# hmmlillian/Neural-Color-Transfer

Hardware: AMD Instinct MI355X
Metric: 700x700 pairs/sec end-to-end L=5->1; PatchMatch HBM GB/s vs peak (higher is better)
Workload: dtype f32

## Files before the change

### neural-color-transfer_amd/csrc/k_vgg.hip

```cpp
#include "nct_internal.h"
#include "nct_device.h"

typedef float f32x16 __attribute__((ext_vector_type(16)));

__global__ void k_vgg_preprocess(const uint8_t* __restrict__ bgr, int stride, float* __restrict__ out, int H, int W) {
    int i = blockIdx.x * blockDim.x + threadIdx.x;
    if (i >= H * W) return;
    int y = i / W, x = i - y * W;
    const uint8_t* p = bgr + (size_t)y * stride + x * 3;
    out[i] = (float)p[0] - 103.939f;
    out[(size_t)H * W + i] = (float)p[1] - 116.779f;
    out[(size_t)2 * H * W + i] = (float)p[2] - 123.68f;
    out[(size_t)3 * H * W + i] = 0.f;
}

struct ConvGeom { int Cin, Cout, H, W, npx_blocks, nblk_n, tiles_x, Ho, Wo; };
#ifndef NCT_CONV_PT1_BELOW
#define NCT_CONV_PT1_BELOW 128
#endif

typedef float f32x32 __attribute__((ext_vector_type(32)));
typedef uint32_t u32x3 __attribute__((ext_vector_type(3)));

template <int WCO, int CT, bool POOL>
__device__ __forceinline__ void conv3x3_mfma2b_body(const float* __restrict__ in, const float* __restrict__ wp ,
                                                    const float* __restrict__ bias, float* __restrict__ out, const ConvGeom& g, int relu, float* __restrict__ out_hwc, int bid) {
    constexpr int WPX = 4 / WCO;
    constexpr int BLK_PX = WPX * 64;
    constexpr int BLK_CO = WCO * 32 * CT;
    const int HW = g.H * g.W;
    int pt, nb;
    {
        const int grp = bid / (8 * g.nblk_n), rem = bid - grp * 8 * g.nblk_n;
        nb = rem >> 3; pt = grp * 8 + (rem & 7);
    }
    if (pt >= g.npx_blocks) return;
    const int wave = threadIdx.x >> 6, lane = threadIdx.x & 63;
    const int half = lane >> 5, l31 = lane & 31;
    const int wco = wave % WCO, wpx = wave / WCO;
    const int m0 = nb * BLK_CO + wco * 32 * CT;
    int y, x, tile_y = 0, tile_x = 0; bool live;
    if constexpr (POOL) {
        const int wt = pt * WPX + wpx;
        tile_y = wt / g.tiles_x; tile_x = wt - tile_y * g.tiles_x;
        y = 2 * tile_y + half; x = 32 * tile_x + l31;
        live = y < g.H && x < g.W;
    } else {
        const int p = pt * BLK_PX + wpx * 64 + lane;
        live = p < HW;
        const int pc = live ? p : 0;
        y = pc / g.W; x = pc - y * g.W;
    }
    const int bias_px = g.H >= 2 ? g.W + 1 : 1;
    const unsigned plane_bytes = (unsigned)HW * 4u, bias_bytes = (unsigned)bias_px * 4u;
    const auto rs = __builtin_amdgcn_make_buffer_rsrc((void*)in, 0, (unsigned)g.Cin * plane_bytes, 0x00020000);

    unsigned voff[3];
    bool rowv[3];
#pragma unroll
    for (int r = 0; r < 3; ++r) {
        voff[r] = live ? (unsigned)(((y + r - 1) * g.W + x - 1 + bias_px) * 4) : 0xFFF00000u;
        rowv[r] = live && (y + r - 1) >= 0 && (y + r - 1) < g.H;
    }
    const bool xl = x > 0, xr = x < g.W - 1;
    auto tapv = [&](int r, int d) { return d == 0 ? (rowv[r] && xl) : (d == 2 ? (rowv[r] && xr) : rowv[r]); };
    bool tm[9];
#pragma unroll
    for (int t = 0; t < 9; ++t) tm[t] = tapv(t / 3, t % 3);

    const float4* ap4 = reinterpret_cast<const float4*>(wp) + (size_t)half * g.Cout + m0 + l31;
    const float* ap1 = wp + (size_t)16 * g.Cout + (size_t)half * g.Cout + m0 + l31;
    unsigned soff = plane_bytes - bias_bytes;

    f32x32 acc0 = {0}, acc1 = {0};
    struct ASet { float4 q0, q1; float s8; };
    struct BSet { u32x3 r[2][3]; };
    ASet a0x, a1x, a0y, a1y; BSet bx, by;
    auto bload = [&](unsigned so, int r) { return __builtin_amdgcn_raw_buffer_load_b96(rs, voff[r], so, 0); };
#ifndef NCT_CONV_TIMING_SKIP
#define NCT_CONV_TIMING_SKIP 0
#endif
    auto load_pair = [&](ASet& a0, ASet& a1, BSet& b) {
        constexpr bool LA = !(NCT_CONV_TIMING_SKIP & 1), LB = !(NCT_CONV_TIMING_SKIP & 2);
        if constexpr (LA) {
            a0.q0 = ap4[0]; a0.q1 = ap4[(size_t)2 * g.Cout]; a0.s8 = ap1[0];
            if constexpr (CT == 2) { a1.q0 = ap4[32]; a1.q1 = ap4[(size_t)2 * g.Cout + 32]; a1.s8 = ap1[32]; }
        }
        if constexpr (LB) {
#pragma unroll
            for (int r = 0; r < 3; ++r) { b.r[0][r] = bload(soff - plane_bytes, r); b.r[1][r] = bload(soff, r); }
        }
        ap4 += (size_t)18 * g.Cout / 4;
        ap1 += (size_t)18 * g.Cout;
        soff += 2u * plane_bytes;
    };
    auto aval = [](const ASet& a, int s) -> float {
        switch (s) { case 0: return a.q0.x; case 1: return a.q0.y; case 2: return a.q0.z; case 3: return a.q0.w;
                     case 4: return a.q1.x; case 5: return a.q1.y; case 6: return a.q1.z; case 7: return a.q1.w; default: return a.s8; }
    };
    auto mma_pair = [&](const ASet& a0, const ASet& a1, const BSet& b) {
#pragma unroll
        for (int k = 0; k < 18; ++k) {
            const int ci = k / 9, t = k - 9 * ci, r = t / 3, d = t - 3 * r, s = k >> 1;
            const float bv = tm[t] ? __uint_as_float(b.r[ci][r][d]) : 0.f;
            if (k & 1) {
                acc0 = __builtin_amdgcn_mfma_f32_32x32x1f32(aval(a0, s), bv, acc0, 1, 1, 0);
                if constexpr (CT == 2) acc1 = __builtin_amdgcn_mfma_f32_32x32x1f32(aval(a1, s), bv, acc1, 1, 1, 0);
            } else {
                acc0 = __builtin_amdgcn_mfma_f32_32x32x1f32(aval(a0, s), bv, acc0, 1, 0, 0);
                if constexpr (CT == 2) acc1 = __builtin_amdgcn_mfma_f32_32x32x1f32(aval(a1, s), bv, acc1, 1, 0, 0);
            }
        }
    };
#ifndef NCT_CONV_SCHED
#define NCT_CONV_SCHED 0
#endif
    auto interleave = [] {
        if constexpr (NCT_CONV_SCHED == 2) return;
        if constexpr (CT == 2) {
#pragma unroll
            for (int i = 0; i < 12; ++i) {
                __builtin_amdgcn_sched_group_barrier(0x008, NCT_CONV_SCHED == 1 ? 1 : 2, 0);
                __builtin_amdgcn_sched_group_barrier(0x020, 1, 0);
                __builtin_amdgcn_sched_group_barrier(0x008, NCT_CONV_SCHED == 1 ? 2 : 1, 0);
            }
        } else {
#pragma unroll
            for (int i = 0; i < 9; ++i) {
                __builtin_amdgcn_sched_group_barrier(0x008, 1, 0);
                __builtin_amdgcn_sched_group_barrier(0x020, 1, 0);
                __builtin_amdgcn_sched_group_barrier(0x008, 1, 0);
            }
        }
    };
    {
        a0x.q0 = ap4[0]; a0x.q1 = ap4[(size_t)2 * g.Cout]; a0x.s8 = ap1[0];
        if constexpr (CT == 2) { a1x.q0 = ap4[32]; a1x.q1 = ap4[(size_t)2 * g.Cout + 32]; a1x.s8 = ap1[32]; }
        ap4 += (size_t)18 * g.Cout / 4;
        ap1 += (size_t)18 * g.Cout;
#pragma unroll
        for (int r = 0; r < 3; ++r) {
            const unsigned v0 = voff[r] - bias_bytes + (xl ? 0u : 4u);
            u32x3 t = __builtin_amdgcn_raw_buffer_load_b96(rs, v0, 0, 0);
            if (!xl) { t.z = t.y; t.y = t.x; }
            bx.r[0][r] = t;
            bx.r[1][r] = __builtin_amdgcn_raw_buffer_load_b96(rs, voff[r], soff, 0);
        }
        soff += 2u * plane_bytes;
    }
    int c2 = 0;
    for (; c2 + 4 <= g.Cin; c2 += 4) {
        load_pair(a0y, a1y, by);
        mma_pair(a0x, a1x, bx);
        interleave();
        __builtin_amdgcn_sched_barrier(0);
        if (c2 + 4 >= g.Cin) { ap4 -= (size_t)18 * g.Cout / 4; ap1 -= (size_t)18 * g.Cout; soff -= 2u * plane_bytes; }
        load_pair(a0x, a1x, bx);
        mma_pair(a0y, a1y, by);
        interleave();
        __builtin_amdgcn_sched_barrier(0);
    }
    if (c2 < g.Cin) mma_pair(a0x, a1x, bx);

    if constexpr (POOL) {
        const int xx = 32 * tile_x + l31, y0 = 2 * tile_y;
        const bool ok0 = y0 < g.H && xx < g.W, ok1 = y0 + 1 < g.H && xx < g.W;
        const size_t po = (size_t)tile_y * g.Wo + (xx >> 1), pn = (size_t)g.Ho * g.Wo;
        const bool writer = ok0 && !(l31 & 1);
        auto pool4 = [&](float top, float bot) {
            top = ok0 ? top : -3.402823466e+38f; bot = ok1 ? bot : -3.402823466e+38f;
            const float top_r = dpp_rot<0xB1>(top), bot_r = dpp_rot<0xB1>(bot);
            float m = -3.402823466e+38f;
            m = top > m ? top : m; m = top_r > m ? top_r : m; m = bot > m ? bot : m; m = bot_r > m ? bot_r : m;
            return m;
        };
#pragma unroll
        for (int r = 0; r < 16; ++r) {
            const int co0 = m0 + (r & 3) + 8 * (r >> 2) + 4 * half;
            const float bb0 = bias[co0];
            float t0 = acc0[r] + bb0, u0 = acc0[16 + r] + bb0;
            if (relu) { t0 = fmaxf(t0, 0.f); u0 = fmaxf(u0, 0.f); }
            const float m0v = pool4(t0, u0);
            if (writer) out[(size_t)co0 * pn + po] = m0v;
            if constexpr (CT == 2) {
                const float bb1 = bias[co0 + 32];
                float t1 = acc1[r] + bb1, u1 = acc1[16 + r] + bb1;
                if (relu) { t1 = fmaxf(t1, 0.f); u1 = fmaxf(u1, 0.f); }
                const float m1v = pool4(t1, u1);
                if (writer) out[(size_t)(co0 + 32) * pn + po] = m1v;
            }
        }
    } else {
        const int pw = pt * BLK_PX + wpx * 64;
        if (out_hwc) {
#pragma unroll
            for (int b = 0; b < 2; ++b) {
                const int pp = pw + 32 * b + l31;
                if (pp < HW) {
                    float* dst = out_hwc + (size_t)pp * g.Cout + m0 + 4 * half;
#pragma unroll
                    for (int gq = 0; gq < 4; ++gq) {
                        float4 v0, v1;
                        float* e0 = &v0.x; float* e1 = &v1.x;
#pragma unroll
                        for (int j = 0; j < 4; ++j) {
                            const int row = j + 8 * gq + 4 * half;
                            float t0 = acc0[16 * b + 4 * gq + j] + bias[m0 + row];
                            if (relu) t0 = fmaxf(t0, 0.f);
                            e0[j] = t0;
                            if constexpr (CT == 2) { float t1 = acc1[16 * b + 4 * gq + j] + bias[m0 + 32 + row]; if (relu) t1 = fmaxf(t1, 0.f); e1[j] = t1; }
                        }
                        *reinterpret_cast<float4*>(dst + 8 * gq) = v0;
                        if constexpr (CT == 2) *reinterpret_cast<float4*>(dst + 32 + 8 * gq) = v1;
                    }
                }
            }
        }
        if (out)
#pragma unroll
        for (int b = 0; b < 2; ++b) {
            const int pp = pw + 32 * b + l31;
            const bool lv = pp < HW;
#pragma unroll
            for (int r = 0; r < 16; ++r) {
                const int row = (r & 3) + 8 * (r >> 2) + 4 * half;
                const int co0 = m0 + row;
                float v0 = acc0[16 * b + r] + bias[co0];
                if (relu) v0 = fmaxf(v0, 0.f);
                if (lv) out[(size_t)co0 * HW + pp] = v0;
                if constexpr (CT == 2) {
                    float v1 = acc1[16 * b + r] + bias[co0 + 32];
                    if (relu) v1 = fmaxf(v1, 0.f);
                    if (lv) out[(size_t)(co0 + 32) * HW + pp] = v1;
                }
            }
        }
    }
}

bool nctk_conv3x3_pool_fits(int H, int W) {
    const long t2 = (long)cdiv(W, 32) * cdiv(H, 2), t1 = cdiv(H * W, 64);
    return t2 * 100 <= t1 * 104;
}

template <int WCO, int CT, bool POOL>
__global__ __launch_bounds__(256) __attribute__((amdgpu_waves_per_eu(3, 3))) void k_conv3x3_mfma2b(const float* __restrict__ in, const float* __restrict__ wp, const float* __restrict__ bias,
                                                        float* __restrict__ out, ConvGeom g, int relu, float* __restrict__ out_hwc) {
    conv3x3_mfma2b_body<WCO, CT, POOL>(in, wp, bias, out, g, relu, out_hwc, (int)blockIdx.x);
}
template <int WCO, int CT>
__global__ __launch_bounds__(256) __attribute__((amdgpu_waves_per_eu(3, 3))) void k_conv3x3_mfma2b_pair(const float* __restrict__ in1, const float* __restrict__ in2, const float* __restrict__ wp,
                                                        const float* __restrict__ bias, float* __restrict__ out1, float* __restrict__ out2, ConvGeom g1, ConvGeom g2, int nblocks1, int relu,
                                                        float* __restrict__ hwc1, float* __restrict__ hwc2) {
    const bool second = (int)blockIdx.x >= nblocks1;
    conv3x3_mfma2b_body<WCO, CT, false>(second ? in2 : in1, wp, bias, second ? out2 : out1, second ? g2 : g1, relu, second ? hwc2 : hwc1, second ? (int)blockIdx.x - nblocks1 : (int)blockIdx.x);
}
int nctk_conv3x3(nct_ctx* ctx, hipStream_t s, const float* in, const float* wp, const float* bias, float* out,
                 int Cin, int Cout, int H, int W, int relu, int pool, float* out_hwc) {
    NCT_REQUIRE(out || out_hwc, "conv3x3: no output");
    NCT_REQUIRE(!(pool && out_hwc), "conv3x3: the channel-last output exists for un-pooled layers only");
    NCT_REQUIRE((Cin & 1) == 0 && (Cout & 63) == 0, "conv3x3: Cin=%d must be even (pad) and Cout=%d a multiple of 64", Cin, Cout);
    NCT_REQUIRE((size_t)Cin * H * W * 4 < ((size_t)1 << 32), "conv3x3: input of %d x %d x %d floats exceeds the 4 GB a buffer descriptor addresses", Cin, H, W);
    const int WCO = (Cout % 128 == 0) ? 2 : 1;
    const int tiles_x = cdiv(W, 32), ntiles = pool ? tiles_x * cdiv(H, 2) : cdiv(H * W, 64);
    const int full_blocks = cdiv(ntiles, 4 / WCO) * (Cout / (64 * WCO));
    const int Ho = (H - 1) / 2 + 1, Wo = (W - 1) / 2 + 1;
#define NCT_CONV_LAUNCH(wco, ct, wpx, nblk_n_)                                                                                                    \
    do {                                                                                                                                          \
        ConvGeom g{Cin, Cout, H, W, cdiv(ntiles, wpx), nblk_n_, tiles_x, Ho, Wo};                                                                  \
        const int nblocks = cdiv(g.npx_blocks, 8) * 8 * g.nblk_n;                                                                                 \
        if (pool) hipLaunchKernelGGL((k_conv3x3_mfma2b<wco, ct, true>), dim3(nblocks), dim3(256), 0, s, in, wp, bias, out, g, relu, (float*)nullptr);             \
        else      hipLaunchKernelGGL((k_conv3x3_mfma2b<wco, ct, false>), dim3(nblocks), dim3(256), 0, s, in, wp, bias, out, g, relu, out_hwc);            \
    } while (0)
    if (full_blocks >= NCT_CONV_PT1_BELOW) {
        if (WCO == 2) NCT_CONV_LAUNCH(2, 2, 2, Cout / 128);
        else          NCT_CONV_LAUNCH(1, 2, 4, Cout / 64);
    } else if (Cout % 128 == 0) NCT_CONV_LAUNCH(4, 1, 1, Cout / 128);
    else                        NCT_CONV_LAUNCH(2, 1, 2, Cout / 64);
#undef NCT_CONV_LAUNCH
    NCT_LAUNCH_CHECK();
    return 0;
}

int nctk_conv3x3_pair(nct_ctx* ctx, hipStream_t s, const float* in1, int H1, int W1, const float* in2, int H2, int W2, const float* wp, const float* bias,
                      float* out1, float* out2, int Cin, int Cout, int relu, float* hwc1, float* hwc2) {
    auto small = [&](int H, int W) {
        const int WCO = (Cout % 128 == 0) ? 2 : 1;
        return cdiv(cdiv(H * W, 64), 4 / WCO) * (Cout / (64 * WCO)) < NCT_CONV_PT1_BELOW;
    };
    const bool ok = (Cin & 1) == 0 && (Cout & 63) == 0 && small(H1, W1) && small(H2, W2) && (size_t)Cin * H1 * W1 * 4 < ((size_t)1 << 32) && (size_t)Cin * H2 * W2 * 4 < ((size_t)1 << 32) &&
                    (out1 || hwc1) && (out2 || hwc2) && ctx->conv_pair != 0;
    if (!ok) {
        int rc = nctk_conv3x3(ctx, s, in1, wp, bias, out1, Cin, Cout, H1, W1, relu, 0, hwc1); if (rc) return rc;
        return nctk_conv3x3(ctx, s, in2, wp, bias, out2, Cin, Cout, H2, W2, relu, 0, hwc2);
    }
    const int nt1 = cdiv(H1 * W1, 64), nt2 = cdiv(H2 * W2, 64);
#define NCT_CONV_PAIR(wco, ct, wpx, nblk_n_)                                                                                                      \
    do {                                                                                                                                          \
        ConvGeom g1{Cin, Cout, H1, W1, cdiv(nt1, wpx), nblk_n_, 0, 0, 0}, g2{Cin, Cout, H2, W2, cdiv(nt2, wpx), nblk_n_, 0, 0, 0};                 \
        const int nb1 = cdiv(g1.npx_blocks, 8) * 8 * g1.nblk_n, nb2 = cdiv(g2.npx_blocks, 8) * 8 * g2.nblk_n;                                     \
        hipLaunchKernelGGL((k_conv3x3_mfma2b_pair<wco, ct>), dim3(nb1 + nb2), dim3(256), 0, s, in1, in2, wp, bias, out1, out2, g1, g2, nb1, relu, hwc1, hwc2); \
    } while (0)
    if (Cout % 128 == 0) NCT_CONV_PAIR(4, 1, 1, Cout / 128);
    else                 NCT_CONV_PAIR(2, 1, 2, Cout / 64);
#undef NCT_CONV_PAIR
    NCT_LAUNCH_CHECK();
    return 0;
}

__global__ void k_maxpool2x2(const float* __restrict__ in, float* __restrict__ out, int C, int H, int W, int Ho, int Wo) {
    size_t i = (size_t)blockIdx.x * blockDim.x + threadIdx.x;
    if (i >= (size_t)C * Ho * Wo) return;
    const int px = (int)(i % Wo); const size_t t = i / Wo; const int py = (int)(t % Ho); const int c = (int)(t / Ho);
    const int hs = py * 2, ws = px * 2, he = min(hs + 2, H), we = min(ws + 2, W);
    const float* p = in + (size_t)c * H * W;
    float m = -3.402823466e+38f;
    for (int y = hs; y < he; ++y)
        for (int x = ws; x < we; ++x) { const float v = p[(size_t)y * W + x]; m = v > m ? v : m; }
    out[i] = m;
}

int nctk_maxpool2x2(nct_ctx* ctx, hipStream_t s, const float* in, float* out, int C, int H, int W) {
    const int Ho = (H - 2 + 1) / 2 + 1, Wo = (W - 2 + 1) / 2 + 1;
    const size_t n = (size_t)C * Ho * Wo;
    hipLaunchKernelGGL(k_maxpool2x2, dim3((unsigned)((n + 255) / 256)), dim3(256), 0, s, in, out, C, H, W, Ho, Wo);
    NCT_LAUNCH_CHECK();
    return 0;
}

int nctk_vgg_preprocess(nct_ctx* ctx, hipStream_t s, const uint8_t* bgr, int stride, float* out, int H, int W) {
    hipLaunchKernelGGL(k_vgg_preprocess, dim3(cdiv(H * W, 256)), dim3(256), 0, s, bgr, stride, out, H, W);
    NCT_LAUNCH_CHECK();
    return 0;
}

__global__ void k_pack_weights(const float* __restrict__ w, float* __restrict__ wp, int Cout, int Cin, int Cin_pad) {
    size_t i = (size_t)blockIdx.x * blockDim.x + threadIdx.x;
    if (i >= (size_t)Cin_pad * 9 * Cout) return;
    const int co = (int)(i % Cout); const int k = (int)(i / Cout);
    const int ci = k / 9, tap = k - ci * 9;
    const float v = ci < Cin ? w[((size_t)co * Cin + ci) * 9 + tap] : 0.f;
    const int P = ci >> 1, k18 = (ci & 1) * 9 + tap, s_ = k18 >> 1, h = k18 & 1;
    const size_t base = (size_t)P * 18 * Cout;
    const size_t dst = s_ < 8 ? base + (size_t)(s_ >> 2) * 8 * Cout + ((size_t)h * Cout + co) * 4 + (s_ & 3)
                              : base + (size_t)16 * Cout + (size_t)h * Cout + co;
    wp[dst] = v;
}

int nctk_pack_weights(nct_ctx* ctx, hipStream_t s, const float* w, float* wp, int Cout, int Cin, int Cin_pad) {
    const size_t n = (size_t)Cin_pad * 9 * Cout;
    hipLaunchKernelGGL(k_pack_weights, dim3((unsigned)((n + 255) / 256)), dim3(256), 0, s, w, wp, Cout, Cin, Cin_pad);
    NCT_LAUNCH_CHECK();
    return 0;
}
```

Baseline: 15.76.

## Deepen conv3x3 MFMA load pipeline to configurable depth with buffer-load weights

Replaces the two-stage ping-pong prefetch in the 3x3 conv MFMA kernel with a D-stage register ring (default 3), so loads for pair p+D-1 are issued while pair p is multiplied. Weight fetches move from pointer arithmetic to buffer-descriptor loads with computed offsets, and a clamp replaces the end-of-loop pointer rewind. Occupancy is lowered from 3 to 2 waves per EU to make room for the extra staged registers. The aim is to hide more memory latency, at the cost of fewer resident waves and more register use.

```diff
diff --git a/neural-color-transfer_amd/csrc/k_vgg.hip b/neural-color-transfer_amd/csrc/k_vgg.hip
--- a/neural-color-transfer_amd/csrc/k_vgg.hip
+++ b/neural-color-transfer_amd/csrc/k_vgg.hip
@@ -1,5 +1,7 @@
 #include "nct_internal.h"
 #include "nct_device.h"
+#include <type_traits>
+#include <utility>
 
 typedef float f32x16 __attribute__((ext_vector_type(16)));
 
@@ -22,7 +24,10 @@
 typedef float f32x32 __attribute__((ext_vector_type(32)));
 typedef uint32_t u32x3 __attribute__((ext_vector_type(3)));
 
-template <int WCO, int CT, bool POOL>
+template <typename F, int... J> __device__ __forceinline__ void static_for_(F&& f, std::integer_sequence<int, J...>) { (f(std::integral_constant<int, J>{}), ...); }
+template <int N, typename F> __device__ __forceinline__ void static_for(F&& f) { static_for_(f, std::make_integer_sequence<int, N>{}); }
+
+template <int WCO, int CT, bool POOL, int D>
 __device__ __forceinline__ void conv3x3_mfma2b_body(const float* __restrict__ in, const float* __restrict__ wp ,
                                                     const float* __restrict__ bias, float* __restrict__ out, const ConvGeom& g, int relu, float* __restrict__ out_hwc, int bid) {
     constexpr int WPX = 4 / WCO;
@@ -68,47 +73,57 @@
 #pragma unroll
     for (int t = 0; t < 9; ++t) tm[t] = tapv(t / 3, t % 3);
 
-    const float4* ap4 = reinterpret_cast<const float4*>(wp) + (size_t)half * g.Cout + m0 + l31;
-    const float* ap1 = wp + (size_t)16 * g.Cout + (size_t)half * g.Cout + m0 + l31;
-    unsigned soff = plane_bytes - bias_bytes;
+    const int npairs = g.Cin >> 1;
+    const unsigned wpair_bytes = 72u * (unsigned)g.Cout;
+    const auto wrs = __builtin_amdgcn_make_buffer_rsrc((void*)wp, 0, (unsigned)npairs * wpair_bytes, 0x00020000);
+    const unsigned wq = (unsigned)(half * g.Cout + m0 + l31) * 16u;
+    const unsigned w8 = (unsigned)(half * g.Cout + m0 + l31) * 4u + 64u * (unsigned)g.Cout;
+    const unsigned wq1 = 32u * (unsigned)g.Cout;
 
     f32x32 acc0 = {0}, acc1 = {0};
     struct ASet { float4 q0, q1; float s8; };
-    struct BSet { u32x3 r[2][3]; };
-    ASet a0x, a1x, a0y, a1y; BSet bx, by;
-    auto bload = [&](unsigned so, int r) { return __builtin_amdgcn_raw_buffer_load_b96(rs, voff[r], so, 0); };
+    struct OSet { ASet a[CT]; u32x3 b[2][3]; };
+    OSet st[D];
+    auto wload4 = [&](unsigned vo, unsigned so) { return __builtin_bit_cast(float4, __builtin_amdgcn_raw_buffer_load_b128(wrs, vo, so, 0)); };
+    auto wload1 = [&](unsigned vo, unsigned so) { return __uint_as_float(__builtin_amdgcn_raw_buffer_load_b32(wrs, vo, so, 0)); };
+    auto aload = [&](ASet& a, int t, unsigned so) {
+        a.q0 = wload4(wq + 512u * t, so); a.q1 = wload4(wq + wq1 + 512u * t, so); a.s8 = wload1(w8 + 128u * t, so);
+    };
 #ifndef NCT_CONV_TIMING_SKIP
 #define NCT_CONV_TIMING_SKIP 0
 #endif
-    auto load_pair = [&](ASet& a0, ASet& a1, BSet& b) {
+    auto load_pair = [&](OSet& o, int p) {
         constexpr bool LA = !(NCT_CONV_TIMING_SKIP & 1), LB = !(NCT_CONV_TIMING_SKIP & 2);
+        p = min(p, npairs - 1);
         if constexpr (LA) {
-            a0.q0 = ap4[0]; a0.q1 = ap4[(size_t)2 * g.Cout]; a0.s8 = ap1[0];
-            if constexpr (CT == 2) { a1.q0 = ap4[32]; a1.q1 = ap4[(size_t)2 * g.Cout + 32]; a1.s8 = ap1[32]; }
+            const unsigned so = (unsigned)p * wpair_bytes;
+#pragma unroll
+            for (int t = 0; t < CT; ++t) aload(o.a[t], t, so);
         }
         if constexpr (LB) {
-#pragma unroll
-            for (int r = 0; r < 3; ++r) { b.r[0][r] = bload(soff - plane_bytes, r); b.r[1][r] = bload(soff, r); }
-        }
-        ap4 += (size_t)18 * g.Cout / 4;
-        ap1 += (size_t)18 * g.Cout;
-        soff += 2u * plane_bytes;
+            const unsigned so = (unsigned)(2 * p + 1) * plane_bytes - bias_bytes;
+#pragma unroll
+            for (int r = 0; r < 3; ++r) {
+                o.b[0][r] = __builtin_amdgcn_raw_buffer_load_b96(rs, voff[r], so - plane_bytes, 0);
+                o.b[1][r] = __builtin_amdgcn_raw_buffer_load_b96(rs, voff[r], so, 0);
+            }
+        }
     };
     auto aval = [](const ASet& a, int s) -> float {
         switch (s) { case 0: return a.q0.x; case 1: return a.q0.y; case 2: return a.q0.z; case 3: return a.q0.w;
                      case 4: return a.q1.x; case 5: return a.q1.y; case 6: return a.q1.z; case 7: return a.q1.w; default: return a.s8; }
     };
-    auto mma_pair = [&](const ASet& a0, const ASet& a1, const BSet& b) {
+    auto mma_pair = [&](const OSet& o) {
 #pragma unroll
         for (int k = 0; k < 18; ++k) {
             const int ci = k / 9, t = k - 9 * ci, r = t / 3, d = t - 3 * r, s = k >> 1;
-            const float bv = tm[t] ? __uint_as_float(b.r[ci][r][d]) : 0.f;
+            const float bv = tm[t] ? __uint_as_float(o.b[ci][r][d]) : 0.f;
             if (k & 1) {
-                acc0 = __builtin_amdgcn_mfma_f32_32x32x1f32(aval(a0, s), bv, acc0, 1, 1, 0);
-                if constexpr (CT == 2) acc1 = __builtin_amdgcn_mfma_f32_32x32x1f32(aval(a1, s), bv, acc1, 1, 1, 0);
+                acc0 = __builtin_amdgcn_mfma_f32_32x32x1f32(aval(o.a[0], s), bv, acc0, 1, 1, 0);
+                if constexpr (CT == 2) acc1 = __builtin_amdgcn_mfma_f32_32x32x1f32(aval(o.a[CT - 1], s), bv, acc1, 1, 1, 0);
             } else {
-                acc0 = __builtin_amdgcn_mfma_f32_32x32x1f32(aval(a0, s), bv, acc0, 1, 0, 0);
-                if constexpr (CT == 2) acc1 = __builtin_amdgcn_mfma_f32_32x32x1f32(aval(a1, s), bv, acc1, 1, 0, 0);
+                acc0 = __builtin_amdgcn_mfma_f32_32x32x1f32(aval(o.a[0], s), bv, acc0, 1, 0, 0);
+                if constexpr (CT == 2) acc1 = __builtin_amdgcn_mfma_f32_32x32x1f32(aval(o.a[CT - 1], s), bv, acc1, 1, 0, 0);
             }
         }
     };
@@ -134,33 +149,28 @@
         }
     };
     {
-        a0x.q0 = ap4[0]; a0x.q1 = ap4[(size_t)2 * g.Cout]; a0x.s8 = ap1[0];
-        if constexpr (CT == 2) { a1x.q0 = ap4[32]; a1x.q1 = ap4[(size_t)2 * g.Cout + 32]; a1x.s8 = ap1[32]; }
-        ap4 += (size_t)18 * g.Cout / 4;
-        ap1 += (size_t)18 * g.Cout;
+#pragma unroll
+        for (int t = 0; t < CT; ++t) aload(st[0].a[t], t, 0u);
 #pragma unroll
         for (int r = 0; r < 3; ++r) {
             const unsigned v0 = voff[r] - bias_bytes + (xl ? 0u : 4u);
             u32x3 t = __builtin_amdgcn_raw_buffer_load_b96(rs, v0, 0, 0);
             if (!xl) { t.z = t.y; t.y = t.x; }
-            bx.r[0][r] = t;
-            bx.r[1][r] = __builtin_amdgcn_raw_buffer_load_b96(rs, voff[r], soff, 0);
-        }
-        soff += 2u * plane_bytes;
-    }
-    int c2 = 0;
-    for (; c2 + 4 <= g.Cin; c2 += 4) {
-        load_pair(a0y, a1y, by);
-        mma_pair(a0x, a1x, bx);
-        interleave();
-        __builtin_amdgcn_sched_barrier(0);
-        if (c2 + 4 >= g.Cin) { ap4 -= (size_t)18 * g.Cout / 4; ap1 -= (size_t)18 * g.Cout; soff -= 2u * plane_bytes; }
-        load_pair(a0x, a1x, bx);
-        mma_pair(a0y, a1y, by);
-        interleave();
-        __builtin_amdgcn_sched_barrier(0);
-    }
-    if (c2 < g.Cin) mma_pair(a0x, a1x, bx);
+            st[0].b[0][r] = t;
+            st[0].b[1][r] = __builtin_amdgcn_raw_buffer_load_b96(rs, voff[r], plane_bytes - bias_bytes, 0);
+        }
+        static_for<D - 2>([&](auto j) { load_pair(st[j + 1], j + 1); });
+    }
+    int c = 0;
+    for (; c + D <= npairs; c += D) {
+        static_for<D>([&](auto j) {
+            load_pair(st[(j + D - 1) % D], c + j + D - 1);
+            mma_pair(st[j]);
+            interleave();
+            __builtin_amdgcn_sched_barrier(0);
+        });
+    }
+    static_for<D - 1>([&](auto j) { if (c + j < npairs) mma_pair(st[j]); });
 
     if constexpr (POOL) {
         const int xx = 32 * tile_x + l31, y0 = 2 * tile_y;
@@ -243,17 +253,21 @@
     return t2 * 100 <= t1 * 104;
 }
 
+#ifndef NCT_CONV_DEPTH
+#define NCT_CONV_DEPTH 3
+#endif
+
 template <int WCO, int CT, bool POOL>
-__global__ __launch_bounds__(256) __attribute__((amdgpu_waves_per_eu(3, 3))) void k_conv3x3_mfma2b(const float* __restrict__ in, const float* __restrict__ wp, const float* __restrict__ bias,
+__global__ __launch_bounds__(256) __attribute__((amdgpu_waves_per_eu(2, 2))) void k_conv3x3_mfma2b(const float* __restrict__ in, const float* __restrict__ wp, const float* __restrict__ bias,
                                                         float* __restrict__ out, ConvGeom g, int relu, float* __restrict__ out_hwc) {
-    conv3x3_mfma2b_body<WCO, CT, POOL>(in, wp, bias, out, g, relu, out_hwc, (int)blockIdx.x);
+    conv3x3_mfma2b_body<WCO, CT, POOL, NCT_CONV_DEPTH>(in, wp, bias, out, g, relu, out_hwc, (int)blockIdx.x);
 }
 template <int WCO, int CT>
-__global__ __launch_bounds__(256) __attribute__((amdgpu_waves_per_eu(3, 3))) void k_conv3x3_mfma2b_pair(const float* __restrict__ in1, const float* __restrict__ in2, const float* __restrict__ wp,
+__global__ __launch_bounds__(256) __attribute__((amdgpu_waves_per_eu(2, 2))) void k_conv3x3_mfma2b_pair(const float* __restrict__ in1, const float* __restrict__ in2, const float* __restrict__ wp,
                                                         const float* __restrict__ bias, float* __restrict__ out1, float* __restrict__ out2, ConvGeom g1, ConvGeom g2, int nblocks1, int relu,
                                                         float* __restrict__ hwc1, float* __restrict__ hwc2) {
     const bool second = (int)blockIdx.x >= nblocks1;
-    conv3x3_mfma2b_body<WCO, CT, false>(second ? in2 : in1, wp, bias, second ? out2 : out1, second ? g2 : g1, relu, second ? hwc2 : hwc1, second ? (int)blockIdx.x - nblocks1 : (int)blockIdx.x);
+    conv3x3_mfma2b_body<WCO, CT, false, NCT_CONV_DEPTH>(second ? in2 : in1, wp, bias, second ? out2 : out1, second ? g2 : g1, relu, second ? hwc2 : hwc1, second ? (int)blockIdx.x - nblocks1 : (int)blockIdx.x);
 }
 int nctk_conv3x3(nct_ctx* ctx, hipStream_t s, const float* in, const float* wp, const float* bias, float* out,
                  int Cin, int Cout, int H, int W, int relu, int pool, float* out_hwc) {
@@ -261,6 +275,7 @@
     NCT_REQUIRE(!(pool && out_hwc), "conv3x3: the channel-last output exists for un-pooled layers only");
     NCT_REQUIRE((Cin & 1) == 0 && (Cout & 63) == 0, "conv3x3: Cin=%d must be even (pad) and Cout=%d a multiple of 64", Cin, Cout);
     NCT_REQUIRE((size_t)Cin * H * W * 4 < ((size_t)1 << 32), "conv3x3: input of %d x %d x %d floats exceeds the 4 GB a buffer descriptor addresses", Cin, H, W);
+    NCT_REQUIRE((size_t)Cin * 9 * Cout * 4 < ((size_t)1 << 32), "conv3x3: packed weights of %d x %d channels exceed the 4 GB a buffer descriptor addresses", Cin, Cout);
     const int WCO = (Cout % 128 == 0) ? 2 : 1;
     const int tiles_x = cdiv(W, 32), ntiles = pool ? tiles_x * cdiv(H, 2) : cdiv(H * W, 64);
     const int full_blocks = cdiv(ntiles, 4 / WCO) * (Cout / (64 * WCO));
@@ -288,7 +303,7 @@
         const int WCO = (Cout % 128 == 0) ? 2 : 1;
         return cdiv(cdiv(H * W, 64), 4 / WCO) * (Cout / (64 * WCO)) < NCT_CONV_PT1_BELOW;
     };
-    const bool ok = (Cin & 1) == 0 && (Cout & 63) == 0 && small(H1, W1) && small(H2, W2) && (size_t)Cin * H1 * W1 * 4 < ((size_t)1 << 32) && (size_t)Cin * H2 * W2 * 4 < ((size_t)1 << 32) &&
+    const bool ok = (Cin & 1) == 0 && (Cout & 63) == 0 && small(H1, W1) && small(H2, W2) && (size_t)Cin * H1 * W1 * 4 < ((size_t)1 << 32) && (size_t)Cin * H2 * W2 * 4 < ((size_t)1 << 32) && (size_t)Cin * 9 * Cout * 4 < ((size_t)1 << 32) &&
                     (out1 || hwc1) && (out2 || hwc2) && ctx->conv_pair != 0;
     if (!ok) {
         int rc = nctk_conv3x3(ctx, s, in1, wp, bias, out1, Cin, Cout, H1, W1, relu, 0, hwc1); if (rc) return rc;
```

New measurement: 15.83 (median of 6 runs). About the same (+0.4%).
